# ZeayW/Multimodal-fusion-based-Pre-routing-Timing-Prediction-

Hardware: AMD Instinct MI355X
Metric: train-step samples/sec (higher is better)
Workload: dtype bf16; 1 GPU; config B: 8 designs/step/GPU, 65536-node netlist, 64 levels, 256x256 tile, 1350 endpoints/design, UNet(max), bf16 operands / fp32 accumulate on the MFMA-bound contractions; U-Net activations and their gradients stored bf16, netlist tensors, statistics, parameters and gradients fp32; nodes=65536, levels=64, tile=256, endpoints_per_design=1350, cone_pruning=False, parallelism=dp1 (designs sharded, one all-reduce of the flat gradient per step), launch=one HIP graph replay per step (Adam inside)

## Files before the change

multimodal-fusion-based-pre-routing-timing-prediction-_amd/csrc/mlp_feat.hip:

```cpp
#include <stdlib.h>
#include "mlp_tile_bf16.h"
#include "tr_read.h"

namespace mmft {

int launch_slab_reduce(const float* slabs, int splits, long long elems, float* out, int accumulate, hipStream_t st);

__device__ __forceinline__ unsigned short mf_bf16(float v) { return (unsigned short)(pack_bf16(v, 0.f) & 0xffff); }

__device__ __forceinline__ bf16x8 mf_pack8(const float* v) {
  u32x4 p = {pack_bf16(v[0], v[1]), pack_bf16(v[2], v[3]), pack_bf16(v[4], v[5]), pack_bf16(v[6], v[7])};
  return __builtin_bit_cast(bf16x8, p);
}

__device__ __forceinline__ bf16x8 mf_w1_frag(const float* __restrict__ w1, int fin, int col, int k0) {
  float v[8];
#pragma unroll
  for (int t = 0; t < 8; ++t) v[t] = k0 + t < fin ? w1[(long long)col * fin + k0 + t] : 0.f;
  return mf_pack8(v);
}

struct FeatFwdArgs {
  const float* x;
  long long ldx;
  int row0, n, fin;
  const float *w1, *b1, *w2, *b2;
  float* out;
  long long ldout;
  int relu_out;
};

template <int KS>
__global__ void __launch_bounds__(512) mlp2_feat_fwd_kernel(FeatFwdArgs a) {
  constexpr int BM = 64, RT = BM / 16, XS = KS * 32 + 8, HS = L2_HD + 8;
  __shared__ __attribute__((aligned(16))) unsigned short xs[BM * XS];
  __shared__ __attribute__((aligned(16))) unsigned short hs[BM * HS];
  const int tid = threadIdx.x, lane = tid & 63, wave = tid >> 6;
  const int r16 = lane & 15, q = lane >> 4;
  bf16x8 w1f[2][KS], w2f[8];
#pragma unroll
  for (int j = 0; j < 2; ++j)
#pragma unroll
    for (int ks = 0; ks < KS; ++ks) w1f[j][ks] = mf_w1_frag(a.w1, a.fin, wave * 32 + j * 16 + r16, ks * 32 + q * 8);
#pragma unroll
  for (int ks = 0; ks < 8; ++ks) w2f[ks] = mf_pack8(a.w2 + (long long)(wave * 16 + r16) * L2_HD + ks * 32 + q * 8);
  const int nn2 = wave * 16 + q * 4;
  const f32x4 b2v = *reinterpret_cast<const f32x4*>(a.b2 + nn2);
  f32x4 b1v[2];
#pragma unroll
  for (int j = 0; j < 2; ++j) b1v[j] = *reinterpret_cast<const f32x4*>(a.b1 + wave * 32 + j * 16 + q * 4);
  constexpr int NXE = BM * KS * 32 / 512;
  float xr[NXE];
  auto request = [&](int tile) {
#pragma unroll
    for (int k = 0; k < NXE; ++k) {
      const int e = tid + k * 512, r = e / (KS * 32), kk = e % (KS * 32);
      const int m = tile * BM + r;
      xr[k] = (m < a.n && kk < a.fin) ? a.x[(long long)(a.row0 + m) * a.ldx + kk] : 0.f;
    }
  };
  const int ntiles = (a.n + BM - 1) / BM;
  if ((int)blockIdx.x < ntiles) request(blockIdx.x);
  for (int tile = blockIdx.x; tile < ntiles; tile += gridDim.x) {
    const int m0 = tile * BM;
#pragma unroll
    for (int k = 0; k < NXE; ++k) {
      const int e = tid + k * 512;
      xs[(e / (KS * 32)) * XS + e % (KS * 32)] = mf_bf16(xr[k]);
    }
    __syncthreads();
    if (tile + (int)gridDim.x < ntiles) request(tile + gridDim.x);
    f32x4 acc1[RT][2];
    tile_layer1<KS, RT>(acc1, w1f, xs, XS, r16, q);
#pragma unroll
    for (int i = 0; i < RT; ++i)
#pragma unroll
      for (int j = 0; j < 2; ++j) st_bf16x4(hs + (i * 16 + r16) * HS + wave * 32 + j * 16 + q * 4, relu4(acc1[i][j] + b1v[j]));
    __syncthreads();
    f32x4 acc2[RT];
#pragma unroll
    for (int i = 0; i < RT; ++i) acc2[i] = tile_layer2(w2f, hs, HS, r16, q, i);
#pragma unroll
    for (int i = 0; i < RT; ++i) {
      const int m = m0 + i * 16 + r16;
      if (m >= a.n) continue;
      f32x4 v = acc2[i] + b2v;
      if (a.relu_out) v = relu4(v);
      *reinterpret_cast<f32x4*>(a.out + (long long)(a.row0 + m) * a.ldout + nn2) = v;
    }
    __syncthreads();
  }
}

struct FeatBwdArgs {
  const float* g;
  long long ldg;
  const float* x;
  long long ldx;
  int row0, n, fin;
  const float *w1, *b1, *w2;
  float* slabs;
  long long slab;
};

template <int KS>
__global__ void __launch_bounds__(512) mlp2_feat_bwd_kernel(FeatBwdArgs a) {
  constexpr int BM = 32, KP = KS * 32, XS = KP + 16, GS = L2_D2 + 16, HS = L2_HD + 16, KB = KP / 16;
  extern __shared__ __attribute__((aligned(16))) unsigned short lds[];
  unsigned short* xs = lds;
  unsigned short* gs = xs + BM * XS;
  unsigned short* hs = gs + BM * GS;
  unsigned short* ds = hs + BM * HS;
  f32x4(*gred)[32] = reinterpret_cast<f32x4(*)[32]>(hs);
  const int tid = threadIdx.x, lane = tid & 63, wave = tid >> 6;
  const int r16 = lane & 15, q = lane >> 4;
  const int trr = tr_lane_row(lane), trc = tr_lane_col(lane);
  const f32x4 zero = {0.f, 0.f, 0.f, 0.f};

  bf16x8 w1f[2][KS], w2tf[2][4];
  f32x4 b1v[2];
#pragma unroll
  for (int j = 0; j < 2; ++j) {
    const int col = wave * 32 + j * 16 + r16;
#pragma unroll
    for (int ks = 0; ks < KS; ++ks) w1f[j][ks] = mf_w1_frag(a.w1, a.fin, col, ks * 32 + q * 8);
#pragma unroll
    for (int ks = 0; ks < 4; ++ks) {
      float v[8];
#pragma unroll
      for (int t = 0; t < 8; ++t) v[t] = a.w2[(long long)(ks * 32 + q * 8 + t) * L2_HD + col];
      w2tf[j][ks] = mf_pack8(v);
    }
    b1v[j] = *reinterpret_cast<const f32x4*>(a.b1 + wave * 32 + j * 16 + q * 4);
  }
  f32x4 dw2[2][8], dw1[2][KB], dsum[2], gsum = zero;
#pragma unroll
  for (int j = 0; j < 2; ++j) {
    dsum[j] = zero;
#pragma unroll
    for (int d = 0; d < 8; ++d) dw2[j][d] = zero;
#pragma unroll
    for (int k = 0; k < KB; ++k) dw1[j][k] = zero;
  }

  const int ntiles = (a.n + BM - 1) / BM;
  constexpr int NXE = BM * KP / 512;
  f32x4 gr[2];
  float xr[NXE];
  auto request = [&](int tile) {
    const int m0 = tile * BM;
#pragma unroll
    for (int it = 0; it < 2; ++it) {
      const int e = tid + it * 512, r = e >> 5, c = (e & 31) * 4;
      gr[it] = m0 + r < a.n ? *reinterpret_cast<const f32x4*>(a.g + (long long)(a.row0 + m0 + r) * a.ldg + c) : zero;
    }
#pragma unroll
    for (int k = 0; k < NXE; ++k) {
      const int e = tid + k * 512, r = e / KP, kk = e % KP;
      xr[k] = (m0 + r < a.n && kk < a.fin) ? a.x[(long long)(a.row0 + m0 + r) * a.ldx + kk] : 0.f;
    }
  };
  if ((int)blockIdx.x < ntiles) request(blockIdx.x);
  for (int tile = blockIdx.x; tile < ntiles; tile += gridDim.x) {
#pragma unroll
    for (int it = 0; it < 2; ++it) {
      const int e = tid + it * 512, r = e >> 5, c = (e & 31) * 4;
      const f32x4 v = gr[it];
      gsum += v;
      const unsigned lo = pack_bf16(v.x, v.y), hi = pack_bf16(v.z, v.w);
      *reinterpret_cast<unsigned long long*>(gs + r * GS + c) = ((unsigned long long)hi << 32) | lo;
    }
#pragma unroll
    for (int k = 0; k < NXE; ++k) {
      const int e = tid + k * 512, r = e / KP, kk = e % KP;
      xs[r * XS + kk] = mf_bf16(xr[k]);
    }
    __syncthreads();
    if (tile + (int)gridDim.x < ntiles) request(tile + gridDim.x);
    __syncthreads();
#pragma unroll
    for (int i = 0; i < 2; ++i) {
      f32x4 acc1[2] = {zero, zero}, acc3[2] = {zero, zero};
#pragma unroll
      for (int ks = 0; ks < KS; ++ks) {
        const bf16x8 xf = *reinterpret_cast<const bf16x8*>(xs + (i * 16 + r16) * XS + ks * 32 + q * 8);
#pragma unroll
        for (int j = 0; j < 2; ++j) acc1[j] = __builtin_amdgcn_mfma_f32_16x16x32_bf16(w1f[j][ks], xf, acc1[j], 0, 0, 0);
      }
#pragma unroll
      for (int ks = 0; ks < 4; ++ks) {
        const bf16x8 gf = *reinterpret_cast<const bf16x8*>(gs + (i * 16 + r16) * GS + ks * 32 + q * 8);
#pragma unroll
        for (int j = 0; j < 2; ++j) acc3[j] = __builtin_amdgcn_mfma_f32_16x16x32_bf16(w2tf[j][ks], gf, acc3[j], 0, 0, 0);
      }
      const int m = i * 16 + r16;
#pragma unroll
      for (int j = 0; j < 2; ++j) {
        const int nn = wave * 32 + j * 16 + q * 4;
        f32x4 hv = acc1[j] + b1v[j], dh = acc3[j];
#pragma unroll
        for (int t = 0; t < 4; ++t) {
          hv[t] = hv[t] > 0.f ? hv[t] : 0.f;
          dh[t] = hv[t] > 0.f ? dh[t] : 0.f;
        }
        dsum[j] += dh;
        const unsigned hl = pack_bf16(hv.x, hv.y), hh = pack_bf16(hv.z, hv.w);
        const unsigned dl = pack_bf16(dh.x, dh.y), dhh = pack_bf16(dh.z, dh.w);
        *reinterpret_cast<unsigned long long*>(hs + m * HS + nn) = ((unsigned long long)hh << 32) | hl;
        *reinterpret_cast<unsigned long long*>(ds + m * HS + nn) = ((unsigned long long)dhh << 32) | dl;
      }
    }
    __syncthreads();
#pragma unroll
    for (int j = 0; j < 2; ++j) {
      const int col0 = wave * 32 + j * 16;
      const bf16x8 hf = __builtin_bit_cast(bf16x8, tr_read_pair(hs + trr * HS + col0 + trc, 16 * HS));
      const bf16x8 df = __builtin_bit_cast(bf16x8, tr_read_pair(ds + trr * HS + col0 + trc, 16 * HS));
#pragma unroll
      for (int d = 0; d < 8; ++d) {
        const bf16x8 gf = __builtin_bit_cast(bf16x8, tr_read_pair(gs + trr * GS + d * 16 + trc, 16 * GS));
        dw2[j][d] = __builtin_amdgcn_mfma_f32_16x16x32_bf16(hf, gf, dw2[j][d], 0, 0, 0);
      }
#pragma unroll
      for (int k = 0; k < KB; ++k) {
        const bf16x8 xf = __builtin_bit_cast(bf16x8, tr_read_pair(xs + trr * XS + k * 16 + trc, 16 * XS));
        dw1[j][k] = __builtin_amdgcn_mfma_f32_16x16x32_bf16(df, xf, dw1[j][k], 0, 0, 0);
      }
    }
    __syncthreads();
  }

  float* sl = a.slabs + (long long)blockIdx.x * a.slab;
  float* s_dw1 = sl;
  float* s_db1 = s_dw1 + (long long)L2_HD * a.fin;
  float* s_dw2 = s_db1 + L2_HD;
  float* s_db2 = s_dw2 + (long long)L2_D2 * L2_HD;
#pragma unroll
  for (int j = 0; j < 2; ++j) {
    const int colq = wave * 32 + j * 16 + q * 4;
#pragma unroll
    for (int d = 0; d < 8; ++d) *reinterpret_cast<f32x4*>(s_dw2 + (long long)(d * 16 + r16) * L2_HD + colq) = dw2[j][d];
#pragma unroll
    for (int k = 0; k < KB; ++k) {
      const int kk = k * 16 + r16;
      if (kk < a.fin) {
#pragma unroll
        for (int t = 0; t < 4; ++t) s_dw1[(long long)(colq + t) * a.fin + kk] = dw1[j][k][t];
      }
    }
    f32x4 v = dsum[j];
#pragma unroll
    for (int o = 1; o < 16; o <<= 1) {
#pragma unroll
      for (int t = 0; t < 4; ++t) v[t] += __shfl_xor(v[t], o, 64);
    }
    if (r16 == 0) *reinterpret_cast<f32x4*>(s_db1 + colq) = v;
  }
  __syncthreads();
  gred[tid >> 5][tid & 31] = gsum;
  __syncthreads();
  if (tid < 32) {
    f32x4 v = gred[0][tid];
    for (int p = 1; p < 16; ++p) v += gred[p][tid];
    *reinterpret_cast<f32x4*>(s_db2 + tid * 4) = v;
  }
}

template <int KS>
constexpr int feat_bwd_lds() {
  constexpr int BM = 32, KP = KS * 32, XS = KP + 16, GS = L2_D2 + 16, HS = L2_HD + 16;
  return (BM * XS + BM * GS + 2 * BM * HS) * 2;
}

static inline long long feat_slab(int fin) { return (long long)L2_HD * fin + L2_HD + (long long)L2_D2 * L2_HD + L2_D2; }
static inline int feat_bwd_grid(int n) {
  int tiles = cdiv(n, 32);
  static int cap = getenv("MMFT_FEAT_BWD_GRID") ? atoi(getenv("MMFT_FEAT_BWD_GRID")) : 192;
  if (cap < 1) cap = 1;
  return tiles < cap ? (tiles < 1 ? 1 : tiles) : cap;
}

}

using namespace mmft;

extern "C" int mmft_mlp2_feat_fwd_bf16(const float* x, long long ldx, int row0, int n, int fin, const float* w1, const float* b1,
                                       const float* w2, const float* b2, float* out, long long ldout, int relu_out, int device,
                                       void* stream) {
  MMFT_REQUIRE(x && w1 && b1 && w2 && b2 && out, "mlp2_feat_fwd_bf16: null pointer");
  MMFT_REQUIRE(n >= 0 && row0 >= 0 && fin >= 1 && fin <= 64 && ldx >= fin, "mlp2_feat_fwd_bf16: bad sizes (fin <= 64)");
  MMFT_REQUIRE(ldout % 4 == 0 && aligned16(out) && aligned16(w2) && aligned16(b1) && aligned16(b2),
               "mlp2_feat_fwd_bf16: out / w2 / biases must be 16-byte aligned");
  if (n == 0) return MMFT_OK;
  DeviceGuard dg(device);
  FeatFwdArgs a{x, ldx, row0, n, fin, w1, b1, w2, b2, out, ldout, relu_out};
  const double fl = 2.0 * n * ((double)fin * L2_HD + (double)L2_HD * L2_D2), by = 4.0 * n * ((double)fin + L2_D2);
  int grid = cdiv(n, 64);
  if (grid > 768) grid = 768;
  if (fin <= 32)
    MMFT_LAUNCH("mlp2_feat_fwd_kernel", fl, by, mlp2_feat_fwd_kernel<1>, dim3(grid), dim3(512), (hipStream_t)stream, a);
  else
    MMFT_LAUNCH("mlp2_feat_fwd_kernel", fl, by, mlp2_feat_fwd_kernel<2>, dim3(grid), dim3(512), (hipStream_t)stream, a);
  return check_launch("mlp2_feat_fwd_bf16");
}

extern "C" long long mmft_mlp2_feat_bwd_workspace_bytes(int n, int fin) {
  if (n <= 0 || fin < 1 || fin > 64) return 0;
  return (long long)feat_bwd_grid(n) * feat_slab(fin) * 4;
}

extern "C" int mmft_mlp2_feat_bwd_bf16(const float* g, long long ldg, const float* x, long long ldx, int row0, int n, int fin,
                                       const float* w1, const float* b1, const float* w2, float* dw1, float* db1, float* dw2,
                                       float* db2, int accumulate, float* workspace, long long workspace_bytes, int device,
                                       void* stream) {
  MMFT_REQUIRE(g && x && w1 && b1 && w2 && dw1 && db1 && dw2 && db2, "mlp2_feat_bwd_bf16: null pointer");
  MMFT_REQUIRE(n > 0 && row0 >= 0 && fin >= 1 && fin <= 64 && ldx >= fin && ldg >= L2_D2, "mlp2_feat_bwd_bf16: bad sizes (fin <= 64)");
  MMFT_REQUIRE(ldg % 4 == 0 && aligned16(g) && aligned16(b1), "mlp2_feat_bwd_bf16: g / b1 must be 16-byte aligned");
  MMFT_REQUIRE(workspace && aligned16(workspace) && workspace_bytes >= mmft_mlp2_feat_bwd_workspace_bytes(n, fin),
               "mlp2_feat_bwd_bf16: workspace too small");
  DeviceGuard dg(device);
  hipStream_t st = (hipStream_t)stream;
  const int grid = feat_bwd_grid(n);
  const long long slab = feat_slab(fin);
  FeatBwdArgs a{g, ldg, x, ldx, row0, n, fin, w1, b1, w2, workspace, slab};
  const double fl = 2.0 * n * (2.0 * fin * L2_HD + 2.0 * L2_HD * L2_D2), by = 4.0 * n * ((double)fin + L2_D2);
  static DynLdsOnce once[2];
  int arc = fin <= 32 ? ensure_dyn_lds(once[0], reinterpret_cast<const void*>(&mlp2_feat_bwd_kernel<1>), feat_bwd_lds<1>(), "mlp2_feat_bwd_bf16")
                      : ensure_dyn_lds(once[1], reinterpret_cast<const void*>(&mlp2_feat_bwd_kernel<2>), feat_bwd_lds<2>(), "mlp2_feat_bwd_bf16");
  if (arc) return arc;
  if (fin <= 32)
    MMFT_LAUNCH_LDS("mlp2_feat_bwd_kernel", fl, by, mlp2_feat_bwd_kernel<1>, dim3(grid), dim3(512), feat_bwd_lds<1>(), st, a);
  else
    MMFT_LAUNCH_LDS("mlp2_feat_bwd_kernel", fl, by, mlp2_feat_bwd_kernel<2>, dim3(grid), dim3(512), feat_bwd_lds<2>(), st, a);
  int rc = check_launch("mlp2_feat_bwd_bf16");
  if (rc) return rc;
  if (db1 == dw1 + (long long)L2_HD * fin && dw2 == db1 + L2_HD && db2 == dw2 + (long long)L2_D2 * L2_HD && aligned16(dw1))
    return launch_slab_reduce(workspace, grid, slab, dw1, accumulate, st);
  const long long o1 = (long long)L2_HD * fin, o2 = o1 + L2_HD, o3 = o2 + (long long)L2_D2 * L2_HD;
  const SlabSeg segs[4] = {{workspace, dw1, slab, grid, (int)o1, 1, accumulate ? 1 : 0},
                           {workspace + o1, db1, slab, grid, L2_HD, 1, accumulate ? 1 : 0},
                           {workspace + o2, dw2, slab, grid, L2_D2 * L2_HD, 1, accumulate ? 1 : 0},
                           {workspace + o3, db2, slab, grid, L2_D2, 1, accumulate ? 1 : 0}};
  return launch_slab_reduce_batch(segs, 4, st);
}
```

Measured before the change: 2437 designs/s.

## Stream feature-MLP backward inputs through an async global-to-LDS ring buffer

The feature-MLP backward kernel now prefetches gradient and input tiles with global_load_lds directly into a 4-deep LDS ring, waiting on vmcnt instead of staging through registers. This is meant to hide global-memory latency across several tiles and cut register pressure. The forward kernel splits layer 1 into two half-tiles to shorten accumulator lifetimes, adds launch_bounds(512,4), and lowers its grid cap from 768 to 512. The changes rely on inline asm and m0 manipulation, clamp out-of-range rows to the last valid row, and enlarge LDS use, which may reduce occupancy.

```diff
diff --git a/multimodal-fusion-based-pre-routing-timing-prediction-_amd/csrc/mlp_feat.hip b/multimodal-fusion-based-pre-routing-timing-prediction-_amd/csrc/mlp_feat.hip
--- a/multimodal-fusion-based-pre-routing-timing-prediction-_amd/csrc/mlp_feat.hip
+++ b/multimodal-fusion-based-pre-routing-timing-prediction-_amd/csrc/mlp_feat.hip
@@ -18,6 +18,29 @@
 #pragma unroll
   for (int t = 0; t < 8; ++t) v[t] = k0 + t < fin ? w1[(long long)col * fin + k0 + t] : 0.f;
   return mf_pack8(v);
+}
+
+typedef __attribute__((address_space(3))) void feat_lptr;
+__device__ __forceinline__ unsigned lds_addr(const void* p) {
+  return __builtin_amdgcn_readfirstlane((unsigned)(unsigned long long)(feat_lptr*)p);
+}
+__device__ __forceinline__ void glds16(const float* src, unsigned dst) {
+  unsigned keep;
+  asm volatile("s_mov_b32 %0, m0\n\ts_mov_b32 m0, %2\n\ts_nop 0\n\tglobal_load_lds_dwordx4 %1, off\n\ts_mov_b32 m0, %0"
+               : "=&s"(keep) : "v"(src), "s"(dst) : "memory");
+}
+__device__ __forceinline__ void glds4(const float* src, unsigned dst) {
+  unsigned keep;
+  asm volatile("s_mov_b32 %0, m0\n\ts_mov_b32 m0, %2\n\ts_nop 0\n\tglobal_load_lds_dword %1, off\n\ts_mov_b32 m0, %0"
+               : "=&s"(keep) : "v"(src), "s"(dst) : "memory");
+}
+template <int N>
+__device__ __forceinline__ void wait_vm() { asm volatile("s_waitcnt vmcnt(%0)" ::"n"(N) : "memory"); }
+__device__ __forceinline__ void wait_lds() { asm volatile("s_waitcnt lgkmcnt(0)" ::: "memory"); }
+__device__ __forceinline__ void wg_barrier() {
+  wait_lds();
+  __builtin_amdgcn_s_barrier();
+  asm volatile("" ::: "memory");
 }
 
 struct FeatFwdArgs {
@@ -31,7 +54,7 @@
 };
 
 template <int KS>
-__global__ void __launch_bounds__(512) mlp2_feat_fwd_kernel(FeatFwdArgs a) {
+__global__ void __launch_bounds__(512, 4) mlp2_feat_fwd_kernel(FeatFwdArgs a) {
   constexpr int BM = 64, RT = BM / 16, XS = KS * 32 + 8, HS = L2_HD + 8;
   __shared__ __attribute__((aligned(16))) unsigned short xs[BM * XS];
   __shared__ __attribute__((aligned(16))) unsigned short hs[BM * HS];
@@ -43,6 +66,10 @@
 #pragma unroll
     for (int ks = 0; ks < KS; ++ks) w1f[j][ks] = mf_w1_frag(a.w1, a.fin, wave * 32 + j * 16 + r16, ks * 32 + q * 8);
 #pragma unroll
+  for (int j = 0; j < 2; ++j)
+#pragma unroll
+    for (int ks = 0; ks < KS; ++ks) asm volatile("" : "+v"(w1f[j][ks]));
+#pragma unroll
   for (int ks = 0; ks < 8; ++ks) w2f[ks] = mf_pack8(a.w2 + (long long)(wave * 16 + r16) * L2_HD + ks * 32 + q * 8);
   const int nn2 = wave * 16 + q * 4;
   const f32x4 b2v = *reinterpret_cast<const f32x4*>(a.b2 + nn2);
@@ -70,12 +97,16 @@
     }
     __syncthreads();
     if (tile + (int)gridDim.x < ntiles) request(tile + gridDim.x);
-    f32x4 acc1[RT][2];
-    tile_layer1<KS, RT>(acc1, w1f, xs, XS, r16, q);
-#pragma unroll
-    for (int i = 0; i < RT; ++i)
-#pragma unroll
-      for (int j = 0; j < 2; ++j) st_bf16x4(hs + (i * 16 + r16) * HS + wave * 32 + j * 16 + q * 4, relu4(acc1[i][j] + b1v[j]));
+#pragma unroll
+    for (int h = 0; h < RT / 2; ++h) {
+      f32x4 acc1[2][2];
+      tile_layer1<KS, 2>(acc1, w1f, xs + h * 32 * XS, XS, r16, q);
+#pragma unroll
+      for (int i = 0; i < 2; ++i)
+#pragma unroll
+        for (int j = 0; j < 2; ++j)
+          st_bf16x4(hs + (h * 32 + i * 16 + r16) * HS + wave * 32 + j * 16 + q * 4, relu4(acc1[i][j] + b1v[j]));
+    }
     __syncthreads();
     f32x4 acc2[RT];
 #pragma unroll
@@ -102,6 +133,8 @@
   float* slabs;
   long long slab;
 };
+
+constexpr int FEAT_RING = 4;
 
 template <int KS>
 __global__ void __launch_bounds__(512) mlp2_feat_bwd_kernel(FeatBwdArgs a) {
@@ -144,28 +177,55 @@
   }
 
   const int ntiles = (a.n + BM - 1) / BM;
-  constexpr int NXE = BM * KP / 512;
-  f32x4 gr[2];
-  float xr[NXE];
-  auto request = [&](int tile) {
+  constexpr int NGI = BM * L2_D2 / 4 / 512, NXE = BM * KP / 512, SLOT = BM * L2_D2 + BM * KP, D = FEAT_RING;
+  float* ring = reinterpret_cast<float*>(ds + BM * HS);
+  auto request = [&](int tile, int slot) {
     const int m0 = tile * BM;
-#pragma unroll
-    for (int it = 0; it < 2; ++it) {
+    const unsigned gsl = lds_addr(ring + slot * SLOT + wave * 256), xsl = lds_addr(ring + slot * SLOT + BM * L2_D2 + wave * 64);
+#pragma unroll
+    for (int it = 0; it < NGI; ++it) {
       const int e = tid + it * 512, r = e >> 5, c = (e & 31) * 4;
-      gr[it] = m0 + r < a.n ? *reinterpret_cast<const f32x4*>(a.g + (long long)(a.row0 + m0 + r) * a.ldg + c) : zero;
+      const int m = m0 + r < a.n ? m0 + r : a.n - 1;
+      glds16(a.g + (long long)(a.row0 + m) * a.ldg + c, gsl + it * 512 * 16);
     }
 #pragma unroll
     for (int k = 0; k < NXE; ++k) {
       const int e = tid + k * 512, r = e / KP, kk = e % KP;
-      xr[k] = (m0 + r < a.n && kk < a.fin) ? a.x[(long long)(a.row0 + m0 + r) * a.ldx + kk] : 0.f;
+      const int m = m0 + r < a.n ? m0 + r : a.n - 1;
+      glds4(a.x + (long long)(a.row0 + m) * a.ldx + (kk < a.fin ? kk : 0), xsl + k * 512 * 4);
     }
   };
-  if ((int)blockIdx.x < ntiles) request(blockIdx.x);
+  wait_vm<0>();
+#pragma unroll
+  for (int j = 0; j < 2; ++j) {
+    asm volatile("" : "+v"(b1v[j]));
+#pragma unroll
+    for (int ks = 0; ks < KS; ++ks) asm volatile("" : "+v"(w1f[j][ks]));
+#pragma unroll
+    for (int ks = 0; ks < 4; ++ks) asm volatile("" : "+v"(w2tf[j][ks]));
+  }
+#pragma unroll
+  for (int d = 0; d < D; ++d) request(blockIdx.x + d * gridDim.x, d);
+  int slot = 0;
   for (int tile = blockIdx.x; tile < ntiles; tile += gridDim.x) {
-#pragma unroll
-    for (int it = 0; it < 2; ++it) {
+    const int m0 = tile * BM;
+    const float* gsl = ring + slot * SLOT;
+    const float* xsl = gsl + BM * L2_D2;
+    wait_vm<(D - 1) * (NGI + NXE)>();
+    wg_barrier();
+    f32x4 gv[NGI];
+    float xv[NXE];
+#pragma unroll
+    for (int it = 0; it < NGI; ++it) gv[it] = *reinterpret_cast<const f32x4*>(gsl + (tid + it * 512) * 4);
+#pragma unroll
+    for (int k = 0; k < NXE; ++k) xv[k] = xsl[tid + k * 512];
+    wait_lds();
+    request(tile + D * (int)gridDim.x, slot);
+    slot = slot + 1 == D ? 0 : slot + 1;
+#pragma unroll
+    for (int it = 0; it < NGI; ++it) {
       const int e = tid + it * 512, r = e >> 5, c = (e & 31) * 4;
-      const f32x4 v = gr[it];
+      const f32x4 v = m0 + r < a.n ? gv[it] : zero;
       gsum += v;
       const unsigned lo = pack_bf16(v.x, v.y), hi = pack_bf16(v.z, v.w);
       *reinterpret_cast<unsigned long long*>(gs + r * GS + c) = ((unsigned long long)hi << 32) | lo;
@@ -173,11 +233,9 @@
 #pragma unroll
     for (int k = 0; k < NXE; ++k) {
       const int e = tid + k * 512, r = e / KP, kk = e % KP;
-      xs[r * XS + kk] = mf_bf16(xr[k]);
-    }
-    __syncthreads();
-    if (tile + (int)gridDim.x < ntiles) request(tile + gridDim.x);
-    __syncthreads();
+      xs[r * XS + kk] = mf_bf16((m0 + r < a.n && kk < a.fin) ? xv[k] : 0.f);
+    }
+    wg_barrier();
 #pragma unroll
     for (int i = 0; i < 2; ++i) {
       f32x4 acc1[2] = {zero, zero}, acc3[2] = {zero, zero};
@@ -210,7 +268,7 @@
         *reinterpret_cast<unsigned long long*>(ds + m * HS + nn) = ((unsigned long long)dhh << 32) | dl;
       }
     }
-    __syncthreads();
+    wg_barrier();
 #pragma unroll
     for (int j = 0; j < 2; ++j) {
       const int col0 = wave * 32 + j * 16;
@@ -227,8 +285,9 @@
         dw1[j][k] = __builtin_amdgcn_mfma_f32_16x16x32_bf16(df, xf, dw1[j][k], 0, 0, 0);
       }
     }
-    __syncthreads();
-  }
+  }
+  wait_vm<0>();
+  wg_barrier();
 
   float* sl = a.slabs + (long long)blockIdx.x * a.slab;
   float* s_dw1 = sl;
@@ -269,7 +328,7 @@
 template <int KS>
 constexpr int feat_bwd_lds() {
   constexpr int BM = 32, KP = KS * 32, XS = KP + 16, GS = L2_D2 + 16, HS = L2_HD + 16;
-  return (BM * XS + BM * GS + 2 * BM * HS) * 2;
+  return (BM * XS + BM * GS + 2 * BM * HS) * 2 + FEAT_RING * (BM * L2_D2 + BM * KP) * 4;
 }
 
 static inline long long feat_slab(int fin) { return (long long)L2_HD * fin + L2_HD + (long long)L2_D2 * L2_HD + L2_D2; }
@@ -296,7 +355,7 @@
   FeatFwdArgs a{x, ldx, row0, n, fin, w1, b1, w2, b2, out, ldout, relu_out};
   const double fl = 2.0 * n * ((double)fin * L2_HD + (double)L2_HD * L2_D2), by = 4.0 * n * ((double)fin + L2_D2);
   int grid = cdiv(n, 64);
-  if (grid > 768) grid = 768;
+  if (grid > 512) grid = 512;
   if (fin <= 32)
     MMFT_LAUNCH("mlp2_feat_fwd_kernel", fl, by, mlp2_feat_fwd_kernel<1>, dim3(grid), dim3(512), (hipStream_t)stream, a);
   else
```

After: 2450 designs/s, median of 3. About the same (+0.5%).
